# parklab/emsar

Measured on AMD Instinct MI355X. Metric: EM iterations/s, higher is better.
Workload: dtype f64

## Files before the change

### emsar_amd/csrc/emsar_hip.hip

```cpp
#include <hip/hip_runtime.h>

#include <algorithm>
#include <chrono>
#include <cmath>
#include <cstdio>
#include <cstdlib>
#include <cstring>
#include <new>
#include <numeric>
#include <string>
#include <vector>

#include "../../include/emsar_hip.h"
#include "layout.hpp"
#include "layout_tiled.hpp"
#include "sets.hpp"
#include "boot_rng.hpp"
#include "internal.hpp"
#include "devmem.hpp"
#include "fit_index.hpp"

#include "kernels_common.hpp"
#include "kernels_csr.hpp"
#include "kernels_tiled.hpp"
// ... 586 lines not shown
    return EMSAR_HIP_OK;
}

int emsar_hip_upload_euma(emsar_hip_ctx *ctx, const int32_t *euma, int32_t nfl) {
    if (!ctx || !euma || nfl <= 0) return EMSAR_HIP_ERR_ARG;
    if (!ctx->have_structure) return EMSAR_HIP_ERR_STATE;
    HIPCHK(hipSetDevice(ctx->device));
    ctx->euma = AdjEuma();
    const size_t n = (size_t)ctx->n_rows * (size_t)nfl;
    AdjEuma A;
    HIPCHK(A.d_euma_t.alloc(n));
    HIPCHK(A.d_wf.alloc((size_t)nfl));
    HIPCHK(A.d_adj.alloc((size_t)ctx->n_rows));
    if (n) {
        DevBuf<int32_t> tmp;
        HIPCHK(tmp.alloc(n));
        HIPCHK(hipMemcpyAsync(tmp, euma, n * 4, hipMemcpyHostToDevice, ctx->stream));
        dim3 grid((unsigned)((ctx->n_rows + 63) / 64), (unsigned)((nfl + 63) / 64));
        hipLaunchKernelGGL(k_transpose_i32, grid, dim3(256), 0, ctx->stream, ctx->n_rows, (int)nfl, tmp, A.d_euma_t);
        HIPCHK(hipGetLastError());
        HIPCHK(hipStreamSynchronize(ctx->stream));
    }
    A.nfl = nfl;
    ctx->euma = std::move(A);
    return EMSAR_HIP_OK;
}

int emsar_hip_adj_euma(emsar_hip_ctx *ctx, const double *wf, double *out) {
    if (!ctx || !wf || !out) return EMSAR_HIP_ERR_ARG;
    if (!ctx->have_structure || ctx->euma.nfl <= 0) return EMSAR_HIP_ERR_STATE;
    HIPCHK(hipSetDevice(ctx->device));
    if (ctx->n_rows == 0) return EMSAR_HIP_OK;
    HIPCHK(hipMemcpyAsync(ctx->euma.d_wf, wf, (size_t)ctx->euma.nfl * 8, hipMemcpyHostToDevice, ctx->stream));
    hipLaunchKernelGGL(k_adj_euma, dim3((unsigned)((ctx->n_rows + 255) / 256)), dim3(256), 0, ctx->stream, ctx->n_rows, (int)ctx->euma.nfl,
                       ctx->euma.d_euma_t, ctx->euma.d_wf, ctx->euma.d_adj);
    HIPCHK(hipGetLastError());
    HIPCHK(hipMemcpyAsync(out, ctx->euma.d_adj, (size_t)ctx->n_rows * 8, hipMemcpyDeviceToHost, ctx->stream));
    HIPCHK(hipStreamSynchronize(ctx->stream));
    return EMSAR_HIP_OK;
}

int emsar_hip_get_info(const emsar_hip_ctx *ctx, emsar_hip_info *o) {
    if (!ctx || !o) return EMSAR_HIP_ERR_ARG;
    if (!ctx->have_structure) return EMSAR_HIP_ERR_STATE;
    memset(o, 0, sizeof(*o));
    o->n_rows = ctx->n_rows; o->nnz = ctx->nnz; o->n_tx = ctx->n_tx; o->device_id = ctx->device;
    o->layout = ctx->layout | ((ctx->layout == EMSAR_LAYOUT_TILED && ctx->lay.TL.merged) ? EMSAR_LAYOUT_FLAG_MERGE_ROWS : 0);
    if (ctx->layout == EMSAR_LAYOUT_TILED) {
        o->n_chunks = ctx->lay.n_tiles; o->n_slices = ctx->tl_n_fslices; o->padded_entries = ctx->tl_fwd_slots;
        o->far_entries = ctx->lay.TL.far_entries; o->window = emsar::kTileDict;
        o->tiled_entries = ctx->lay.TL.tiled_entries; o->tiled_ids = ctx->lay.TL.tiled_ids; o->renumbered = ctx->lay.TL.renum.applied ? 1 : 0;
        o->n_units = ctx->lay.n_units;
    }
    o->bytes_per_pass = ctx->bytes_formula;
    o->stored_bytes_per_pass = stored_bytes(ctx);
    return EMSAR_HIP_OK;
}

int emsar_hip_layout_selfcheck_tiled(int64_t n_rows, int32_t n_tx, const uint64_t *row_ptr, const int32_t *col_idx,
                                     int merge_rows, emsar_hip_info *info_out) {
    try {
        if (emsar::validate_csr(n_rows, n_tx, row_ptr, col_idx) != 0) return EMSAR_HIP_ERR_ARG;
        emsar::TiledLayout L;
        if (emsar::build_tiled(n_rows, n_tx, row_ptr, col_idx, L, merge_rows != 0) != 0) return EMSAR_HIP_ERR_ARG;
        int rc = emsar::check_tiled(L, row_ptr, col_idx);
        if (rc == 0) { emsar::UnitTables U; emsar::build_unit_tables(L, U); rc = emsar::check_unit_tables(L, U); }
        if (info_out) {
            memset(info_out, 0, sizeof(*info_out));
            info_out->n_rows = n_rows; info_out->nnz = L.nnz; info_out->n_tx = n_tx;
            info_out->layout = EMSAR_LAYOUT_TILED | (L.merged ? EMSAR_LAYOUT_FLAG_MERGE_ROWS : 0);
            info_out->n_chunks = (int64_t)L.tiles.size();
            info_out->n_slices = L.n_fslices;
            info_out->padded_entries = L.padded_slots; info_out->far_entries = L.far_entries; info_out->window = emsar::kTileDict;
            info_out->stored_bytes_per_pass = (int64_t)L.fwd.size() * 4 + (int64_t)L.bwd.size() * 4 +
                                              (int64_t)L.far_tid.size() * 4 + (int64_t)L.tiles.size() * 64 + (int64_t)L.left_col.size() * 4;
            info_out->bytes_per_pass = (int64_t)L.single_row.size();
            info_out->tiled_entries = L.tiled_entries; info_out->tiled_ids = L.tiled_ids; info_out->renumbered = L.renum.applied ? 1 : 0;
            info_out->n_units = L.unit_first.empty() ? 0 : (int64_t)L.unit_first.size() - 1;
        }
        return rc == 0 ? EMSAR_HIP_OK : EMSAR_HIP_ERR_ARG - 100 + rc;
    } catch (const std::bad_alloc &) { return EMSAR_HIP_ERR_OOM; }
}

int emsar_hip_sets_selfcheck(int64_t n_rows, int32_t n_tx, const uint64_t *row_ptr, const int32_t *col_idx,
                             const int32_t *row_weight, emsar_hip_sets_info *o) {
    try {
        if (emsar::validate_csr(n_rows, n_tx, row_ptr, col_idx) != 0) return EMSAR_HIP_ERR_ARG;
        if (row_weight) for (int64_t r = 0; r < n_rows; r++) if (row_weight[r] < 0) return EMSAR_HIP_ERR_ARG;
        emsar::ResidentSets S;
        try {
            emsar::build_sets(n_rows, n_tx, row_ptr, col_idx, row_weight, S);
        } catch (const std::bad_alloc &) { return EMSAR_HIP_ERR_OOM; }
        int rc = emsar::check_sets(n_rows, n_tx, row_ptr, col_idx, row_weight, S);
        if (o) {
            memset(o, 0, sizeof(*o));
            o->n_components = S.n_components;
            for (int c = 0; c < emsar::kSetClasses; c++) { o->sets_resident[c] = (int64_t)S.desc[c].size(); o->max_lds_bytes[c] = (int64_t)S.max_lds[c]; }
            o->sets_streamed = S.n_streamed_sets;
            o->tids_closed = S.n_closed_tids; o->tids_resident = S.n_resident_tids; o->tids_streamed = S.n_streamed_tids;
            o->rows_in = S.rows_in; o->rows_stored = S.rows_stored + S.CL.rows_stored;
            o->sets_cluster = S.n_cluster_sets(); o->tids_cluster = S.CL.n_tids; o->max_lds_cluster = (int64_t)S.CL.max_lds;
        }
        return rc == 0 ? EMSAR_HIP_OK : EMSAR_HIP_ERR_ARG - 200 + rc;
    } catch (const std::bad_alloc &) { return EMSAR_HIP_ERR_OOM; }
}

}

#include "solve.hpp"
#include "resample.hpp"
#include "fit.hpp"
```

### emsar_amd/csrc/kernels_tiled.hpp

```cpp
#pragma once

namespace {

#ifndef EMSAR_UE_BATCH
#define EMSAR_UE_BATCH 6
#endif
#ifndef EMSAR_UM_BATCH
#define EMSAR_UM_BATCH 6
#endif
constexpr int kTiledThreads = 256;
constexpr int kRPL = emsar::kRowsPerLane;
constexpr int kTiledWr = emsar::kTileSliceRows + 8;
constexpr int kTiledDictPad = emsar::kDictEntries;
constexpr int kBlk = emsar::kBlk;
constexpr int kTiledLdsDoubles = 2 * kTiledDictPad + emsar::kTileSlices * kTiledWr;

__device__ __forceinline__ double lds_at(const double *base, unsigned byte_off) {
    return *reinterpret_cast<const double *>(reinterpret_cast<const char *>(base) + byte_off);
}
__device__ __forceinline__ unsigned id_off(unsigned dword, int f) { return ((dword >> (10 * f)) & 0x3FFu) << 3; }

typedef int v4i_t __attribute__((ext_vector_type(4)));
__device__ __forceinline__ void load8_clamped(int4 (&q)[8], const int4 *e, int n) {
#pragma unroll
    for (int j = 0; j < 8; j++) {
        const v4i_t t = __builtin_nontemporal_load(reinterpret_cast<const v4i_t *>(e + (size_t)(j < n ? j : n - 1) * 64));
        q[j] = make_int4(t.x, t.y, t.z, t.w);
    }
}

template <int LO>
__device__ __forceinline__ void load4_clamped(int4 (&q)[8], const int4 *e, int n) {
#pragma unroll
    for (int j = LO; j < LO + 4; j++) {
        const v4i_t t = __builtin_nontemporal_load(reinterpret_cast<const v4i_t *>(e + (size_t)(j < n ? j : n - 1) * 64));
        q[j] = make_int4(t.x, t.y, t.z, t.w);
    }
}

typedef __attribute__((address_space(3))) const double lds_cdouble;
__device__ __forceinline__ unsigned lds_byte_addr(const void *p) { return (unsigned)(uintptr_t)p; }
template <int F>
__device__ __forceinline__ unsigned lds_id_addr(unsigned dword, unsigned base ) {
    unsigned a;
    asm("v_bfe_u32 %0, %1, %2, 10\n\tv_lshl_add_u32 %0, %0, 3, %3" : "=v"(a) : "v"(dword), "i"(10 * F), "s"(base));
    return a;
}
__device__ __forceinline__ double lds_ld(unsigned a) { return *reinterpret_cast<lds_cdouble *>(a); }
template <int H>
__device__ __forceinline__ void lds_addr6(const int4 t, unsigned base, unsigned (&a)[6]) {
    const unsigned d0 = (unsigned)(H ? t.z : t.x), d1 = (unsigned)(H ? t.w : t.y);
    a[0] = lds_id_addr<0>(d0, base); a[1] = lds_id_addr<1>(d0, base); a[2] = lds_id_addr<2>(d0, base);
    a[3] = lds_id_addr<0>(d1, base); a[4] = lds_id_addr<1>(d1, base); a[5] = lds_id_addr<2>(d1, base);
}

template <int BATCH = 12, int LO = 0, int HI = 8>
__device__ __forceinline__ void fwd_sum_regs(const int4 (&q)[8], int n, unsigned th_base, double (&S)[kRPL]) {
#pragma unroll
    for (int j = LO; j < HI; j++) {
        if (j < n) {
            if (BATCH == 12) {
                unsigned a0[6], a1[6];
                double v[12];
                lds_addr6<0>(q[j], th_base, a0); lds_addr6<1>(q[j], th_base, a1);
#pragma unroll
                for (int i = 0; i < 6; i++) { v[i] = lds_ld(a0[i]); }
#pragma unroll
                for (int i = 0; i < 6; i++) { v[6 + i] = lds_ld(a1[i]); }
#pragma unroll
                for (int i = 0; i < 12; i++) S[i] += v[i];
            } else {
                unsigned a[6];
                double v[6];
                lds_addr6<0>(q[j], th_base, a);
#pragma unroll
                for (int i = 0; i < 6; i++) v[i] = lds_ld(a[i]);
#pragma unroll
                for (int i = 0; i < 6; i++) S[i] += v[i];
                lds_addr6<1>(q[j], th_base, a);
#pragma unroll
                for (int i = 0; i < 6; i++) v[i] = lds_ld(a[i]);
#pragma unroll
                for (int i = 0; i < 6; i++) S[6 + i] += v[i];
            }
        }
    }
}

__device__ __forceinline__ void tile_acc_add(double *acc_w, unsigned off, double part, double fx) {
    double *p = reinterpret_cast<double *>(reinterpret_cast<char *>(acc_w) + off);
    if (fx != 0.0) lds_add_i64(p, __double2ll_rn(part * *(p - kTiledDictPad) * fx));
    else lds_add_f64(p, part);
}
__device__ __forceinline__ void vm_loads_landed() { __builtin_amdgcn_s_waitcnt(0x0F70); }

struct DTile {
    uint64_t fwd_off, bwd_off;
    uint32_t row_base, far_off;
    int32_t lo;
    uint32_t near_n, far_n, n_slices, follows, wave_of;
    uint32_t k[4], m[4];
};
struct TileWords { uint32_t w[16]; };
static_assert(sizeof(TileWords) == sizeof(Tile), "tile_load reads a Tile as 16 dwords");
static_assert(offsetof(Tile, fwd_off) == 0 && offsetof(Tile, bwd_off) == 8 && offsetof(Tile, row_base) == 16 && offsetof(Tile, far_off) == 20 &&
              offsetof(Tile, coo_off) == 24 && offsetof(Tile, lo) == 28 && offsetof(Tile, near_n) == 32 && offsetof(Tile, far_n) == 34 &&
              offsetof(Tile, n_slices) == 36 && offsetof(Tile, follows) == 38 &&
              offsetof(Tile, wave_of) == 39 && offsetof(Tile, k) == 40 && offsetof(Tile, m) == 48 && offsetof(Tile, coo_n) == 56, "tile_load's field positions");
__device__ __forceinline__ DTile tile_load(const Tile *p ) {
    const TileWords r = *reinterpret_cast<const TileWords *>(p);
    DTile T;
    T.fwd_off = (uint64_t)r.w[0] | (uint64_t)r.w[1] << 32;
    T.bwd_off = (uint64_t)r.w[2] | (uint64_t)r.w[3] << 32;
    T.row_base = r.w[4]; T.far_off = r.w[5]; T.lo = (int32_t)r.w[7];
    T.near_n = r.w[8] & 0xFFFFu; T.far_n = r.w[8] >> 16;
    T.n_slices = r.w[9] & 0xFFFFu; T.follows = (r.w[9] >> 16) & 0xFFu; T.wave_of = r.w[9] >> 24;
#pragma unroll
    for (int s = 0; s < 4; s++) {
        T.k[s] = (r.w[10 + s / 2] >> (16 * (s & 1))) & 0xFFFFu;
        T.m[s] = (r.w[12 + s / 2] >> (16 * (s & 1))) & 0xFFFFu;
    }
    return T;
}

struct BlockDict { double th[kBlk]; int tid[kBlk]; int stid[2]; };
constexpr int kSlotsPerThread = (emsar::kTileDict + kTiledThreads - 1) / kTiledThreads;
static_assert(kSlotsPerThread <= 2, "BlockDict::stid");
static_assert(emsar::kFarMax <= kBlk * (kTiledThreads - emsar::kDictBlocks), "kBlk far entries per thread that owns no near block");
__device__ __forceinline__ void block_dict_far_issue(const int32_t *far, int n, BlockDict &D) {
#pragma unroll
    for (int i = 0; i < kBlk; i++) {
        D.tid[i] = -1;
        const int f = ((int)threadIdx.x - emsar::kDictBlocks) + i * (kTiledThreads - emsar::kDictBlocks);
        if ((int)threadIdx.x >= emsar::kDictBlocks && f < n) D.tid[i] = __builtin_nontemporal_load(&far[f]);
    }
}
template <int MODE>
__device__ __forceinline__ void block_dict_issue(const DTile &T, const double *theta, BlockDict &D) {
    const int near_n = (int)T.near_n, nb = (near_n + kBlk - 1) / kBlk;
    const bool near_thread = (int)threadIdx.x < emsar::kDictBlocks;
#pragma unroll
    for (int i = 0; i < kBlk; i++) {
        D.th[i] = 0.0;
        if (near_thread) {
            D.tid[i] = -1;
            const int d = (int)threadIdx.x * kBlk + i;
            if ((int)threadIdx.x < nb && d < near_n) D.tid[i] = T.lo + d;
        }
        if (MODE != MODE_SCATTER && D.tid[i] >= 0) D.th[i] = theta[D.tid[i]];
    }
#pragma unroll
    for (int j = 0; j < 2; j++) {
        const int sl = (int)threadIdx.x + j * kTiledThreads;
        D.stid[j] = sl < near_n ? T.lo + sl : -1;
    }
}
__device__ __forceinline__ void block_dict_store(const DTile &T, const BlockDict &D, double *th_w, double *acc_w) {
    constexpr int NE = emsar::kBlkEntries;
    const int nb = ((int)T.near_n + kBlk - 1) / kBlk;
    if ((int)threadIdx.x < emsar::kDictBlocks) {
        if ((int)threadIdx.x < nb) {
            double *t = th_w + threadIdx.x * NE, *a = acc_w + threadIdx.x * NE;
            double v[NE];
            v[0] = 0.0;
#pragma unroll
            for (int m = 1; m < NE; m++) {
                const int hi = 31 - __builtin_clz((unsigned)m);
                v[m] = v[m & ~(1 << hi)] + D.th[hi];
            }
            const int sw = EMSAR_SWZ ? (int)(threadIdx.x & (NE - 1)) : 0;
#pragma unroll
            for (int m = 0; m < NE; m++) { t[m ^ sw] = v[m]; a[m] = 0.0; }
        }
    } else {
#pragma unroll
        for (int i = 0; i < kBlk; i++) {
            if (D.tid[i] < 0) continue;
            const int e = NE * nb + ((int)threadIdx.x - emsar::kDictBlocks) + i * (kTiledThreads - emsar::kDictBlocks);
            th_w[e] = D.th[i]; acc_w[e] = 0.0;
        }
    }
}
__device__ __forceinline__ void block_dict_flush(const DTile &T, const BlockDict &D, const double *th_w, const double *acc_w, double *acc, double fx) {
    constexpr int NE = emsar::kBlkEntries;
#pragma unroll
    for (int j = 0; j < 2; j++) {
        const int tid = D.stid[j];
        if (tid < 0) continue;
        const int sl = (int)threadIdx.x + j * kTiledThreads, b = sl / kBlk, i = sl - b * kBlk;
        const double *a = acc_w + b * NE;
        const int sw = EMSAR_SWZ ? (b & (NE - 1)) : 0;
        if (fx != 0.0) {
            const double *t = th_w + b * NE;
            double si = 0.0;
#pragma unroll
            for (int m = 1; m < NE; m++) {
                const double tm = t[m ^ sw];
                if ((m >> i & 1) && tm > 0.0) si += (double)__double_as_longlong(a[m ^ sw]) / tm;
            }
            const long long iv = __double2ll_rn(t[(1 << i) ^ sw] * si);
            if (iv != 0) atomic_add_i64(&acc[tid], iv);
        } else {
            double si = 0.0;
#pragma unroll
            for (int m = 1; m < NE; m++) if (m >> i & 1) si += a[m ^ sw];
            if (si != 0.0) atomic_add_f64(&acc[tid], si);
        }
    }
#ifndef EMSAR_EXP_NO_FAR_FLUSH
    if ((int)threadIdx.x >= emsar::kDictBlocks) {
        const int nb = ((int)T.near_n + kBlk - 1) / kBlk;
#pragma unroll
        for (int i = 0; i < kBlk; i++) {
            if (D.tid[i] < 0) continue;
            const int f = ((int)threadIdx.x - emsar::kDictBlocks) + i * (kTiledThreads - emsar::kDictBlocks), e = NE * nb + f;
            const double v = acc_w[e];
            if (fx != 0.0) { const long long iv = __double_as_longlong(v); if (iv != 0) atomic_add_i64(&acc[D.tid[i]], iv); }
            else if (v != 0.0) atomic_add_f64(&acc[D.tid[i]], v);
        }
    }
#endif
}

template <int BATCH = 12, int LO = 0, int HI = 8>
__device__ __forceinline__ void bwd_sum_regs(const int4 (&q)[8], int n, unsigned ws_base, double *acc_w, unsigned &cur, double &part, double fx) {
#pragma unroll
    for (int j = LO; j < HI; j++) {
        if (j < n) {
            const unsigned col = id_off((unsigned)q[j].x, 0);
            double sum;
            if (BATCH == 12) {
                unsigned a0[6], a1[6];
                double v[12];
                lds_addr6<0>(q[j], ws_base, a0); lds_addr6<1>(q[j], ws_base, a1);
#pragma unroll
                for (int i = 1; i < 6; i++) v[i] = lds_ld(a0[i]);
#pragma unroll
                for (int i = 0; i < 6; i++) v[6 + i] = lds_ld(a1[i]);
                double s0 = v[1] + v[2], s1 = v[3] + v[4], s2 = v[5] + v[6], s3 = v[7] + v[8];
                s0 += v[9]; s1 += v[10]; s2 += v[11];
                sum = (s0 + s1) + (s2 + s3);
            } else {
                unsigned a[6];
                double v[6];
                lds_addr6<0>(q[j], ws_base, a);
#pragma unroll
                for (int i = 1; i < 6; i++) v[i] = lds_ld(a[i]);
                double s0 = v[1] + v[2], s1 = v[3] + v[4];
                s0 += v[5];
                lds_addr6<1>(q[j], ws_base, a);
#pragma unroll
                for (int i = 0; i < 6; i++) v[i] = lds_ld(a[i]);
                s0 += v[0]; s1 += v[1];
                double s2 = v[2] + v[3], s3 = v[4] + v[5];
                sum = (s0 + s1) + (s2 + s3);
            }
            if (col != cur) {
                if (part != 0.0) tile_acc_add(acc_w, cur, part, fx);
                cur = col; part = 0.0;
            }
            part += sum;
        }
    }
}

__device__ __forceinline__ unsigned long long stamp_now() {
    unsigned long long t;
    asm volatile("s_memtime %0\n\ts_waitcnt lgkmcnt(0)" : "=s"(t)::"memory");
    return t;
}

__device__ __forceinline__ unsigned long long stamp_real() {
    unsigned long long t;
    asm volatile("s_memrealtime %0\n\ts_waitcnt lgkmcnt(0)" : "=s"(t)::"memory");
    return t;
}
__device__ __forceinline__ unsigned stamp_place() {
    unsigned hw, xcc;
    asm volatile("s_getreg_b32 %0, hwreg(HW_REG_HW_ID)\n\ts_getreg_b32 %1, hwreg(HW_REG_XCC_ID)" : "=s"(hw), "=s"(xcc));
    return (xcc & 0xFu) << 16 | (hw & 0xFFFFu);
}

struct LlAcc { double v = 0.0, p = 1.0; int e = 0; };
__device__ __forceinline__ double ll_value(const LlAcc &a) { return a.v + (log(a.p) + (double)a.e * 0.6931471805599453094); }
template <int N>
__device__ __forceinline__ double sum_log_rows(const double (&S)[N], double *w_s, int lane) {
    static_assert(N == 12, "rows per lane");
    double h[2];
#pragma unroll
    for (int g = 0; g < 2; g++) {
        double p = 1.0;
#pragma unroll
        for (int i = 6 * g; i < 6 * g + 6; i++) p *= S[i] > 0.0 ? S[i] : 1.0;
        h[g] = p;
    }
    if (h[0] > 1e-140 && h[0] < 1e140 && h[1] > 1e-140 && h[1] < 1e140) return log(h[0] * h[1]);
#pragma unroll
    for (int i = 0; i < N; i++) w_s[64 * i + lane] = S[i];
    double ll = 0.0;
#pragma unroll 1
    for (int i = 0; i < N; i++) { const double v = w_s[64 * i + lane]; if (v > 0.0) ll += log(v); }
    return ll;
// ... 153 lines not shown
        const int n0 = W.k - j0 < 8 ? W.k - j0 : 8;
        if (j0) load8_clamped(A, W.e + (size_t)j0 * 64, n0);
        fwd_sum_regs<EMSAR_UE_BATCH>(A, n0, th_base, S);
    }
    if (WEIGHTED && MODE == MODE_EM_LL) {
#pragma unroll
        for (int i = 0; i < kRPL; i++) w_s[64 * i + lane] = S[i];
        __builtin_amdgcn_fence(__ATOMIC_RELEASE, "wavefront");
        double acc = 0.0;
#pragma unroll 1
        for (int i = 0; i < kRPL; i++) {
            const double s = w_s[64 * i + lane];
            const int ri = __builtin_nontemporal_load(&wgt[slot0 + 64 * i]);
            const bool live = s > 0.0 && ri > 0;
            const double rd = (double)ri;
            w_s[64 * i + lane] = live ? rd / s : 0.0;
            if (live) acc += rd * log(s);
        }
        ll.v += acc;
        __builtin_amdgcn_fence(__ATOMIC_RELEASE, "wavefront");
        __builtin_amdgcn_wave_barrier();
        __builtin_amdgcn_fence(__ATOMIC_ACQUIRE, "wavefront");
        return;
    }
    if (WEIGHTED) {
#pragma unroll
        for (int i = 0; i < kRPL; i++) r[i] = __builtin_nontemporal_load(&wgt[slot0 + 64 * i]);
    }
    if (MODE == MODE_EM_LL && !WEIGHTED) {
#pragma unroll
        for (int i = 0; i < kRPL; i++) {
            const bool pos = S[i] > 0.0;
            ll.p *= pos ? __builtin_amdgcn_frexp_mant(S[i]) : 1.0;
            ll.e += pos ? __builtin_amdgcn_frexp_exp(S[i]) : 0;
        }
        ll.e += __builtin_amdgcn_frexp_exp(ll.p);
        ll.p = __builtin_amdgcn_frexp_mant(ll.p);
    }
#pragma unroll
    for (int i = 0; i < kRPL; i++) {
        const bool live = (S[i] > 0.0) && (r[i] > 0);
        const double ri = WEIGHTED ? (double)r[i] : 1.0;
        w_s[64 * i + lane] = live ? ri / S[i] : 0.0;
        if (MODE == MODE_EM_LL && WEIGHTED && live) ll.v += ri * log(S[i]);
    }
    __builtin_amdgcn_fence(__ATOMIC_RELEASE, "wavefront");
    __builtin_amdgcn_wave_barrier();
    __builtin_amdgcn_fence(__ATOMIC_ACQUIRE, "wavefront");
}
__device__ __forceinline__ void tile_m_step(const TileWave &W, int4 (&B)[8], const double *w_s, double *acc_w, double fx) {
    const unsigned ws_base = __builtin_amdgcn_readfirstlane(lds_byte_addr(w_s));
    unsigned cur = 0xFFFFFFFFu;
    double part = 0.0;
    bwd_sum_regs<EMSAR_UM_BATCH, 0, 4>(B, W.m, ws_base, acc_w, cur, part, fx);
    if (W.m > 8) {
        const int n1 = W.m - 8 < 8 ? W.m - 8 : 8;
        const int4 *b1 = W.b + (size_t)8 * 64;
        __builtin_amdgcn_sched_barrier(0);
        load4_clamped<0>(B, b1, n1);
        __builtin_amdgcn_sched_barrier(0);
        bwd_sum_regs<EMSAR_UM_BATCH, 4, 8>(B, 8, ws_base, acc_w, cur, part, fx);
        __builtin_amdgcn_sched_barrier(0);
        load4_clamped<4>(B, b1, n1);
        __builtin_amdgcn_sched_barrier(0);
        bwd_sum_regs<EMSAR_UM_BATCH, 0, 4>(B, n1, ws_base, acc_w, cur, part, fx);
        bwd_sum_regs<EMSAR_UM_BATCH, 4, 8>(B, n1, ws_base, acc_w, cur, part, fx);
        for (int j0 = 16; j0 < W.m; j0 += 8) {
            const int n0 = W.m - j0 < 8 ? W.m - j0 : 8;
            load8_clamped(B, W.b + (size_t)j0 * 64, n0);
            bwd_sum_regs<EMSAR_UM_BATCH>(B, n0, ws_base, acc_w, cur, part, fx);
        }
    } else bwd_sum_regs<EMSAR_UM_BATCH, 4, 8>(B, W.m, ws_base, acc_w, cur, part, fx);
    if (part != 0.0) tile_acc_add(acc_w, cur, part, fx);
}
struct TileEnv {
    const Tile *tiles; int n_tiles, stride;
    const uint32_t *fwd, *bwd; const int32_t *far_tid, *wgt; const double *theta; double *acc;
    double *th_w, *acc_w, *w_s; int lane, wave; double fx;
};
template <bool WEIGHTED, int MODE, int I, int N>
__device__ __forceinline__ void tiled_stage(const TileEnv &V, int it, const DTile &T, const TileWave &W, int4 (&A)[8], int4 (&B)[8],
                                            BlockDict &D, LlAcc &ll) {
    block_dict_store(T, D, V.th_w, V.acc_w);
    const BlockDict Dcur = D;
    const int in = it + V.stride;
    const bool has_next = (I + 1 < N) && in < V.n_tiles;
    const DTile Tn = tile_load(V.tiles + (has_next ? in : it));
    __syncthreads();
    if (W.has_slice)
        tile_e_step<WEIGHTED, MODE>(W, A, (size_t)T.row_base + (size_t)V.wave * emsar::kTileSliceRows + V.lane, V.wgt, V.th_w, V.w_s, V.lane, ll);
    const TileWave Wn = tile_wave(Tn, V.wave, V.lane, V.fwd, V.bwd);
    if (has_next) {
        if (Wn.has_slice) load8_clamped(A, Wn.e, Wn.k < 8 ? Wn.k : 8);
        block_dict_far_issue(V.far_tid + Tn.far_off, (int)Tn.far_n, D);
        block_dict_issue<MODE>(Tn, V.theta, D);
    }
    if (W.has_slice) tile_m_step(W, B, V.w_s, V.acc_w, V.fx);
    if (has_next && Wn.has_slice && Wn.m > 0) load8_clamped(B, Wn.b, Wn.m < 8 ? Wn.m : 8);
    __syncthreads();
    block_dict_flush(T, Dcur, V.th_w, V.acc_w, V.acc, V.fx);
    if constexpr (I + 1 < N) {
        if (has_next) __syncthreads();
        if (has_next) tiled_stage<WEIGHTED, MODE, I + 1, N>(V, in, Tn, Wn, A, B, D, ll);
    }
}

template <bool WEIGHTED, int MODE, int N>
__global__ __launch_bounds__(kTiledThreads, 4) void k_pass_tiled_multi(const Tile *__restrict__ tiles, int n_tiles, const uint32_t *__restrict__ fwd,
                                                                    const uint32_t *__restrict__ bwd,
                                                                    const int32_t *__restrict__ far_tid, const int32_t *__restrict__ wgt,
                                                                    const double *__restrict__ theta, double *__restrict__ acc,
                                                                    double *__restrict__ ll_out, Fx fx) {
    extern __shared__ __attribute__((aligned(16))) double lds[];
    __shared__ double red[kTiledThreads / 64];
    TileEnv V;
    V.tiles = tiles; V.n_tiles = n_tiles; V.stride = (int)gridDim.x; V.fwd = fwd; V.bwd = bwd; V.far_tid = far_tid; V.wgt = wgt;
    V.theta = theta; V.acc = acc; V.fx = fx.mass;
    V.lane = threadIdx.x & 63;
    V.wave = __builtin_amdgcn_readfirstlane(threadIdx.x >> 6);
    V.th_w = lds; V.acc_w = lds + kTiledDictPad; V.w_s = lds + 2 * kTiledDictPad + V.wave * kTiledWr;
    const DTile T = tile_load(tiles + blockIdx.x);
    const TileWave W = tile_wave(T, V.wave, V.lane, fwd, bwd);
    BlockDict D;
    int4 A[8], B[8];
    block_dict_far_issue(far_tid + T.far_off, (int)T.far_n, D);
    block_dict_issue<MODE>(T, theta, D);
    if (W.has_slice) {
        load8_clamped(A, W.e, W.k < 8 ? W.k : 8);
        if (W.m > 0) load8_clamped(B, W.b, W.m < 8 ? W.m : 8);
    }
    if (V.lane < 8) V.w_s[emsar::kTileSliceRows + V.lane] = 0.0;
    LlAcc ll;
    tiled_stage<WEIGHTED, MODE, 0, N>(V, (int)blockIdx.x, T, W, A, B, D, ll);
    if (MODE == MODE_EM_LL) {
        double t = block_sum<kTiledThreads>(ll_value(ll), red);
        if (threadIdx.x == 0 && t != 0.0) ll_add(ll_out, t, fx.ll);
    }
}

template <bool WEIGHTED, int MODE, bool STAMP = false>
__global__ __launch_bounds__(kTiledThreads, 4) void k_pass_tiled_unit(const Tile *__restrict__ utiles, int stride, const int32_t *__restrict__ far_tid,
                                                                   const uint32_t *__restrict__ fwd, const uint32_t *__restrict__ bwd,
                                                                   
                                                                   const int32_t *__restrict__ wgt, const double *__restrict__ theta,
                                                                   double *__restrict__ acc, double *__restrict__ ll_out, Fx fx,
                                                                   unsigned long long *stamps = nullptr) {
    extern __shared__ __attribute__((aligned(16))) double lds[];
    __shared__ double red[kTiledThreads / 64];
    const int lane = threadIdx.x & 63;
    const int wave = __builtin_amdgcn_readfirstlane(threadIdx.x >> 6);
    double *th_w = lds, *acc_w = lds + kTiledDictPad, *w_s = lds + 2 * kTiledDictPad + wave * kTiledWr;
    unsigned long long ts0 = 0, ts1 = 0, ts2 = 0, te = 0, tm = 0, tr0 = 0;
    if (STAMP) { ts0 = stamp_now(); tr0 = stamp_real(); }
    const Tile *tiles = utiles + (size_t)blockIdx.x * (size_t)stride;
    BlockDict D;
    DTile T = tile_load(tiles);
    block_dict_far_issue(far_tid + T.far_off, (int)T.far_n, D);
    const int dict_near_n = (int)T.near_n, dict_lo = T.lo, dict_far_n = (int)T.far_n;
    const uint32_t dict_far_off = T.far_off;
    TileWave W = tile_wave(T, unit_slice(T, wave), lane, fwd, bwd);
    int4 A[8], B[8];
    load8_clamped(A, W.has_slice ? W.e : reinterpret_cast<const int4 *>(fwd), W.has_slice ? (W.k < 8 ? W.k : 8) : 1);
    block_dict_issue<MODE>(T, theta, D);
    if (lane < 8) w_s[emsar::kTileSliceRows + lane] = 0.0;
    block_dict_store(T, D, th_w, acc_w);
    vm_loads_landed();
    if (STAMP) ts1 = stamp_now();
    __syncthreads();
    if (STAMP) ts2 = stamp_now();
    LlAcc ll;
    int n_done = 0;
    for (int t = 0;; t++) {
        unsigned long long ta = 0, tb = 0;
        if (STAMP) ta = stamp_now();
        if (W.has_slice) {
            load8_clamped(B, W.b, W.m < 8 ? W.m : 8);
            tile_e_step<WEIGHTED, MODE>(W, A, (size_t)T.row_base + (size_t)W.slice * emsar::kTileSliceRows + lane, wgt, th_w, w_s, lane, ll);
        }
        const DTile Tn = tile_load(tiles + (t + 1 < stride ? t + 1 : t));
        const bool more = t + 1 < stride && Tn.n_slices > 0;
        TileWave Wn = tile_wave(Tn, unit_slice(Tn, wave), lane, fwd, bwd);
        if (!more) Wn.has_slice = false;
        if (STAMP) tb = stamp_now();
        if (W.has_slice) {
            load8_clamped(A, Wn.has_slice ? Wn.e : reinterpret_cast<const int4 *>(fwd), Wn.has_slice ? (Wn.k < 8 ? Wn.k : 8) : 1);
            tile_m_step(W, B, w_s, acc_w, fx.mass);
        } else if (Wn.has_slice) load8_clamped(A, Wn.e, Wn.k < 8 ? Wn.k : 8);
        if (STAMP) { const unsigned long long tc = stamp_now(); te += tb - ta; tm += tc - tb; }
        T = Tn; W = Wn;
        n_done = t + 1;
        if (!more) break;
    }
    unsigned long long ts3 = 0, ts4 = 0;
    if (STAMP) ts3 = stamp_now();
    block_dict_far_issue(far_tid + dict_far_off, dict_far_n, D);
    __syncthreads();
    if (STAMP) ts4 = stamp_now();
#pragma unroll
    for (int j = 0; j < 2; j++) {
        const int sl = (int)threadIdx.x + j * kTiledThreads;
        D.stid[j] = sl < dict_near_n ? dict_lo + sl : -1;
    }
    T.near_n = (uint32_t)dict_near_n;
    block_dict_flush(T, D, th_w, acc_w, acc, fx.mass);
    if (STAMP && lane == 0) {
        unsigned long long *o = stamps + ((size_t)blockIdx.x * (kTiledThreads / 64) + wave) * 8;
        o[0] = ts1 - ts0; o[1] = ts2 - ts1; o[2] = te; o[3] = tm; o[4] = ts4 - ts3; o[5] = stamp_now() - ts4; o[6] = n_done; o[7] = ts3 - ts2 - te - tm;
        if (wave == 0) {
            unsigned long long *g = stamps + (size_t)gridDim.x * (kTiledThreads / 64) * 8 + (size_t)blockIdx.x * 4;
            g[0] = tr0; g[1] = stamp_real(); g[2] = stamp_place(); g[3] = (unsigned long long)n_done;
        }
    }
    if (MODE == MODE_EM_LL) {
        double t = block_sum<kTiledThreads>(ll_value(ll), red);
        if (threadIdx.x == 0 && t != 0.0) ll_add(ll_out, t, fx.ll);
    }
}

__global__ __launch_bounds__(256) void k_single_ll(int n, const double *__restrict__ u, const double *__restrict__ theta, double *ll_out, double fx_ll) {
    __shared__ double red[4];
    double s = 0.0;
    for (int t = blockIdx.x * 256 + threadIdx.x; t < n; t += gridDim.x * 256) {
        double x = theta[t], c = u[t];
        if (c > 0.0 && x > 0.0) s += c * log(x);
    }
    double tot = block_sum<256>(s, red);
    if (threadIdx.x == 0 && tot != 0.0) ll_add(ll_out, tot, fx_ll);
}

}
```

### emsar_amd/hip.py

```python
import ctypes as C
import os

import numpy as np

_PKG = os.path.dirname(os.path.abspath(__file__))
_LIB_PATH = os.environ.get("EMSAR_HIP_LIB") or os.path.join(_PKG, "libemsar_hip.so")
_lib = None

LAYOUT_AUTO, LAYOUT_CSR, LAYOUT_TILED = 0, 1, 3
FLAG_MERGE_ROWS = 0x100

SYMBOLS = [
    "emsar_hip_create", "emsar_hip_destroy", "emsar_hip_strerror", "emsar_hip_last_error",
    "emsar_hip_upload_structure", "emsar_hip_upload_sample", "emsar_hip_solve",
    "emsar_hip_reset_theta", "emsar_hip_set_theta", "emsar_hip_get_theta", "emsar_hip_run_passes",
    "emsar_hip_ieuma", "emsar_hip_normalise", "emsar_hip_get_info",
    "emsar_hip_layout_selfcheck_tiled", "emsar_hip_sets_selfcheck", "emsar_hip_upload_euma", "emsar_hip_adj_euma", "emsar_hip_collapse_rows",
    "emsar_hip_set_deterministic", "emsar_hip_bootstrap", "emsar_hip_bootstrap_weights", "emsar_hip_bootstrap_draw_host",
    "emsar_hip_set_gene_map", "emsar_hip_gene_sums", "emsar_hip_bootstrap_genes",
    "emsar_hip_subsample", "emsar_hip_subsample_weights", "emsar_hip_subsample_draw_host",
    "emsar_hip_bootstrap_quantiles", "emsar_hip_quantiles_host",
    "emsar_hip_isoform_usage", "emsar_hip_isoform_usage_host", "emsar_hip_bootstrap_isoforms",
    "emsar_hip_model_fit", "emsar_hip_model_fit_host",
]
# ... 209 lines not shown
    return out[:, 0] if one else out


def isoform_usage_host(gene_of_tx, n_genes, cols, want_dominant=False):
    L = load_library()
    g = _arr(gene_of_tx, np.int32)
    x = _arr(cols, np.float64)
    one = x.ndim == 1
    x = np.ascontiguousarray(np.atleast_2d(x))
    if x.shape[1] != len(g):
        raise ValueError("columns of n_tx values expected")
    usage = np.zeros(x.shape)
    dom = np.zeros((x.shape[0], max(int(n_genes), 1)), dtype=np.int32) if want_dominant else None
    rc = L.emsar_hip_isoform_usage_host(len(g), int(n_genes), _p(g, C.c_int32), x.shape[0], _p(x, C.c_double), _p(usage, C.c_double),
                                        _p(dom, C.c_int32))
    if rc != 0:
        raise EmsarHipError(rc, "isoform_usage_host")
    if not want_dominant:
        return usage[0] if one else usage
    dom = dom[:, :max(int(n_genes), 0)]
    return (usage[0], dom[0]) if one else (usage, dom)


def _fit_buffers(n_rows, n_tx, n_genes, rows, genes):
    res = {k: np.zeros(max(n_tx, 1)) for k in ("tx_chi2", "tx_dev", "tx_miss", "tx_df")}
    res["tx_worst_row"] = np.zeros(max(n_tx, 1), dtype=np.int32)
    if rows:
        res.update({k: np.zeros(max(n_rows, 1)) for k in ("row_mu", "row_chi2", "row_dev")})
    if genes:
        res.update({k: np.zeros(max(n_genes, 1)) for k in ("gene_chi2", "gene_dev", "gene_miss", "gene_df")})
    o = FitOutputs()
    for k, a in res.items():
        setattr(o, k, _p(a, C.c_int32 if k == "tx_worst_row" else C.c_double))
    return res, o


def _fit_result(res, n_rows, n_tx, n_genes, st):
    out = {k: v[:(n_rows if k.startswith("row_") else n_genes if k.startswith("gene_") else n_tx)] for k, v in res.items()}
    out["stats"] = st
    return out


def model_fit_host(n_tx, row_ptr, col_idx, theta, row_weight=None, E=None, rows=False, gene_of_tx=None, n_genes=0, genes=None):
    L = load_library()
    row_ptr, col_idx, th = _arr(row_ptr, np.uint64), _arr(col_idx, np.int32), _arr(theta, np.float64)
    w, e, g = _arr(row_weight, np.int32), _arr(E, np.float64), _arr(gene_of_tx, np.int32)
    n_rows = len(row_ptr) - 1
    for a, n in ((th, n_tx), (w, n_rows), (e, n_rows), (g, n_tx)):
        if a is not None and a.shape != (n,):
            raise ValueError("array of length %d expected" % n)
    want_genes = (g is not None) if genes is None else bool(genes)
    res, o = _fit_buffers(n_rows, n_tx, int(n_genes), rows, want_genes)
    st = FitStats()
    rc = L.emsar_hip_model_fit_host(n_rows, int(n_tx), _p(row_ptr, C.c_uint64), _p(col_idx, C.c_int32), _p(w, C.c_int32), _p(e, C.c_double),
                                    _p(th, C.c_double), int(n_genes), _p(g, C.c_int32), C.byref(o), C.byref(st))
    if rc != 0:
        raise EmsarHipError(rc, "model_fit_host")
    return _fit_result(res, n_rows, int(n_tx), int(n_genes), st)


def layout_selfcheck_tiled(n_tx, row_ptr, col_idx, merge_rows=False):
    L = load_library()
    row_ptr, col_idx = _arr(row_ptr, np.uint64), _arr(col_idx, np.int32)
    info = Info()
    rc = L.emsar_hip_layout_selfcheck_tiled(len(row_ptr) - 1, n_tx, _p(row_ptr, C.c_uint64), _p(col_idx, C.c_int32),
                                            int(merge_rows), C.byref(info))
    if rc != 0:
        raise EmsarHipError(rc, "layout_selfcheck_tiled")
    d = info.as_dict()
    d["folded_single_rows"] = d.pop("bytes_per_pass")
    return d


def debug_pass_kernel(weighted, mode, n_tiles, tiled_multi=1, weighted_unit=1):
    f = load_library().emsar_hip_debug_pass_kernel
    f.argtypes = [C.c_int, C.c_int, C.c_int64, C.c_int, C.c_int, C.c_char_p, C.c_size_t]
    buf = C.create_string_buffer(64)
    rc = f(int(bool(weighted)), int(mode), int(n_tiles), int(tiled_multi), int(weighted_unit), buf, len(buf))
    if rc != 0:
        raise EmsarHipError(rc, "debug_pass_kernel")
    return buf.value.decode()


class EmsarHip:

    def __init__(self, device_id=0):
        self._L = load_library()
        h = C.c_void_p()
        rc = self._L.emsar_hip_create(C.byref(h), device_id)
        if rc != 0:
            raise EmsarHipError(rc, "emsar_hip_create")
        self._h = h
        self.n_tx = 0
        self.n_rows = 0
        self.n_genes = 0

    def close(self):
        if getattr(self, "_h", None):
            self._L.emsar_hip_destroy(self._h)
            self._h = None

    __del__ = close

    def __enter__(self):
        return self

    def __exit__(self, *a):
        self.close()

    def _chk(self, rc, what):
        if rc != 0:
            raise EmsarHipError(rc, what, self._L.emsar_hip_last_error(self._h).decode())

    def upload_structure(self, n_tx, row_ptr, col_idx, layout=LAYOUT_AUTO, merge_rows=False):
        row_ptr, col_idx = _arr(row_ptr, np.uint64), _arr(col_idx, np.int32)
        if merge_rows:
            layout |= FLAG_MERGE_ROWS
        self._chk(self._L.emsar_hip_upload_structure(self._h, len(row_ptr) - 1, n_tx, _p(row_ptr, C.c_uint64),
                                                     _p(col_idx, C.c_int32), layout), "upload_structure")
        self.n_tx = int(n_tx)
        self.n_rows = len(row_ptr) - 1
        self.n_genes = 0

    def upload_sample(self, row_weight=None, row_E=None, den=None):
        w, e, d = _arr(row_weight, np.int32), _arr(row_E, np.float64), _arr(den, np.float64)
        for a, n in ((w, self.n_rows), (e, self.n_rows), (d, self.n_tx)):
            if a is not None and a.shape != (n,):
                raise ValueError("array of length %d expected" % n)
        self._chk(self._L.emsar_hip_upload_sample(self._h, _p(w, C.c_int32), _p(e, C.c_double), _p(d, C.c_double)),
                  "upload_sample")

    def solve(self, max_iter=100000, accel=1, tol=1e-10, abs_floor=1e-6, check_every=8, count_floor=0.0, set_mode=0, zero_cut=0.0, abs_step=0.0,
              newton_after=0):
        p = EmParams(max_iter, accel, tol, abs_floor, check_every, set_mode, count_floor, zero_cut, abs_step, newton_after, 0)
        st = EmStats()
        out = np.zeros(self.n_tx)
        self._chk(self._L.emsar_hip_solve(self._h, C.byref(p), _p(out, C.c_double), C.byref(st)), "solve")
        return out, st

    def bootstrap(self, n, seed, first=0, want_replicates=False, max_iter=100000, accel=1, tol=1e-10, abs_floor=1e-6, check_every=8,
                  count_floor=0.0, set_mode=0, zero_cut=0.0, abs_step=0.0, newton_after=0):
        p = EmParams(max_iter, accel, tol, abs_floor, check_every, set_mode, count_floor, zero_cut, abs_step, newton_after, 0)
        mean, sd, tsd = np.zeros(self.n_tx), np.zeros(self.n_tx), np.zeros(self.n_tx)
        reps = np.zeros((n, self.n_tx)) if (want_replicates and n > 0) else None
        st = BootStats()
        self._chk(self._L.emsar_hip_bootstrap(self._h, C.byref(p), int(seed) & 0xFFFFFFFFFFFFFFFF, int(first), int(n), _p(mean, C.c_double),
                                              _p(sd, C.c_double), _p(tsd, C.c_double), _p(reps, C.c_double), C.byref(st)), "bootstrap")
        return mean, sd, tsd, reps, st

    def set_gene_map(self, gene_of_tx, n_genes):
        g = _arr(gene_of_tx, np.int32)
        if self.n_tx and g.shape != (self.n_tx,):
            raise ValueError("gene_of_tx must have n_tx entries")
        self._chk(self._L.emsar_hip_set_gene_map(self._h, int(n_genes), _p(g, C.c_int32)), "set_gene_map")
        self.n_genes = int(n_genes)

    def gene_sums(self, cols):
        x = _arr(cols, np.float64)
        one = x.ndim == 1
        x = np.ascontiguousarray(np.atleast_2d(x))
        if x.shape[1] != self.n_tx:
            raise ValueError("columns of n_tx values expected")
        out = np.zeros((x.shape[0], max(self.n_genes, 1)))
        self._chk(self._L.emsar_hip_gene_sums(self._h, x.shape[0], _p(x, C.c_double), _p(out, C.c_double)), "gene_sums")
        out = out[:, :self.n_genes]
        return out[0] if one else out
# ... 202 lines not shown
```

Baseline: 9695.

## Spread dictionary build across all threads with quad DPP broadcast and fold masks

Reworks the per-tile LDS dictionary build so every thread loads one near theta and up to three far entries, rather than dedicating a few threads to near blocks and the rest to far entries. Each quad of lanes shares its four thetas through DPP broadcasts and each lane writes four of the sixteen subset sums. The flush reads only the eight subset entries that contain a bit. Far tids are reloaded before the flush instead of being kept in registers across the stage. The aim is to cut the serial subset-sum work and register pressure in the build, in exchange for extra global reloads of far ids and cross-lane DPP traffic.

Measured after the change: 9806 (median of 6 runs). No clear change (+1.1%).

```diff
diff --git a/emsar_amd/csrc/dict_map.hpp b/emsar_amd/csrc/dict_map.hpp
--- /dev/null
+++ b/emsar_amd/csrc/dict_map.hpp
@@ -0,0 +1,37 @@
+#pragma once
+
+namespace emsar {
+namespace dictmap {
+
+constexpr int kThreads = 256;
+constexpr int kSlots = 4;
+constexpr int kEntries = 1 << kSlots;
+constexpr int kLaneEntries = kEntries / kSlots;
+constexpr int kFarPerThread = 3;
+constexpr int kFoldTerms = kEntries / 2;
+
+constexpr int near_blocks(int near_n) { return (near_n + kSlots - 1) / kSlots; }
+constexpr bool builds_near(int x, int nb) { return x < kSlots * nb; }
+constexpr int near_block(int x) { return x / kSlots; }
+constexpr int near_quad(int x) { return x % kSlots; }
+constexpr int built_mask(int q, int l) { return kLaneEntries * q + l; }
+constexpr int table_entry(int b, int m, int sw) { return kEntries * b + (m ^ sw); }
+
+constexpr int far_index(int x, int i) { return x + kThreads * i; }
+constexpr int far_entry(int nb, int f) { return kEntries * nb + f; }
+
+constexpr int fold_mask(int i, int c) { return ((c >> i) << (i + 1)) | (1 << i) | (c & ((1 << i) - 1)); }
+
+constexpr void quad_sums(const double (&th)[kSlots], int q, double (&v)[kLaneEntries]) {
+    const double z = 0.0, s0 = z + th[0], s1 = z + th[1], s01 = s0 + th[1];
+    v[0] = z; v[1] = s0; v[2] = s1; v[3] = s01;
+    for (int l = 0; l < kLaneEntries; l++) {
+        const double with2 = v[l] + th[2];
+        v[l] = (q & 1) ? with2 : v[l];
+        const double with3 = v[l] + th[3];
+        v[l] = (q & 2) ? with3 : v[l];
+    }
+}
+
+}
+}
diff --git a/emsar_amd/csrc/emsar_hip.hip b/emsar_amd/csrc/emsar_hip.hip
--- a/emsar_amd/csrc/emsar_hip.hip
+++ b/emsar_amd/csrc/emsar_hip.hip
@@ -692,6 +692,22 @@
     } catch (const std::bad_alloc &) { return EMSAR_HIP_ERR_OOM; }
 }
 
+int emsar_hip_debug_unit_dicts(int64_t n_rows, int32_t n_tx, const uint64_t *row_ptr, const int32_t *col_idx, int merge_rows,
+                               int32_t *out, int64_t cap, int64_t *n_units) {
+    try {
+        if (!n_units || (cap > 0 && !out) || emsar::validate_csr(n_rows, n_tx, row_ptr, col_idx) != 0) return EMSAR_HIP_ERR_ARG;
+        emsar::TiledLayout L;
+        if (emsar::build_tiled(n_rows, n_tx, row_ptr, col_idx, L, merge_rows != 0) != 0) return EMSAR_HIP_ERR_ARG;
+        const int64_t nu = L.unit_first.empty() ? 0 : (int64_t)L.unit_first.size() - 1;
+        *n_units = nu;
+        for (int64_t u = 0; u < nu && u < cap; u++) {
+            const emsar::Tile &T = L.tiles[L.unit_first[(size_t)u]];
+            out[3 * u] = T.lo; out[3 * u + 1] = (int32_t)T.near_n; out[3 * u + 2] = (int32_t)T.far_n;
+        }
+        return EMSAR_HIP_OK;
+    } catch (const std::bad_alloc &) { return EMSAR_HIP_ERR_OOM; }
+}
+
 int emsar_hip_sets_selfcheck(int64_t n_rows, int32_t n_tx, const uint64_t *row_ptr, const int32_t *col_idx,
                              const int32_t *row_weight, emsar_hip_sets_info *o) {
     try {
diff --git a/emsar_amd/csrc/kernels_tiled.hpp b/emsar_amd/csrc/kernels_tiled.hpp
--- a/emsar_amd/csrc/kernels_tiled.hpp
+++ b/emsar_amd/csrc/kernels_tiled.hpp
@@ -1,4 +1,5 @@
 #pragma once
+#include "dict_map.hpp"
 
 namespace {
 
@@ -123,101 +124,109 @@
     return T;
 }
 
-struct BlockDict { double th[kBlk]; int tid[kBlk]; int stid[2]; };
+namespace dm = emsar::dictmap;
+struct BlockDict { double th; double fth[dm::kFarPerThread]; int ftid[dm::kFarPerThread]; };
 constexpr int kSlotsPerThread = (emsar::kTileDict + kTiledThreads - 1) / kTiledThreads;
-static_assert(kSlotsPerThread <= 2, "BlockDict::stid");
-static_assert(emsar::kFarMax <= kBlk * (kTiledThreads - emsar::kDictBlocks), "kBlk far entries per thread that owns no near block");
+static_assert(kBlk == dm::kSlots && emsar::kBlkEntries == dm::kEntries && kTiledThreads == dm::kThreads, "dict_map.hpp: a block is a quad of lanes");
+static_assert(emsar::kTileDict <= kTiledThreads, "one near slot per thread in the build");
+static_assert(emsar::kFarMax <= dm::kFarPerThread * kTiledThreads, "kFarPerThread far entries per thread");
+#ifndef EMSAR_FAR_NT
+#define EMSAR_FAR_NT 3
+#endif
+template <bool NT = true>
 __device__ __forceinline__ void block_dict_far_issue(const int32_t *far, int n, BlockDict &D) {
 #pragma unroll
-    for (int i = 0; i < kBlk; i++) {
-        D.tid[i] = -1;
-        const int f = ((int)threadIdx.x - emsar::kDictBlocks) + i * (kTiledThreads - emsar::kDictBlocks);
-        if ((int)threadIdx.x >= emsar::kDictBlocks && f < n) D.tid[i] = __builtin_nontemporal_load(&far[f]);
+    for (int i = 0; i < dm::kFarPerThread; i++) {
+        D.ftid[i] = -1;
+        const int f = dm::far_index((int)threadIdx.x, i);
+        if (f < n) D.ftid[i] = NT ? __builtin_nontemporal_load(&far[f]) : far[f];
     }
 }
 template <int MODE>
 __device__ __forceinline__ void block_dict_issue(const DTile &T, const double *theta, BlockDict &D) {
-    const int near_n = (int)T.near_n, nb = (near_n + kBlk - 1) / kBlk;
-    const bool near_thread = (int)threadIdx.x < emsar::kDictBlocks;
-#pragma unroll
-    for (int i = 0; i < kBlk; i++) {
-        D.th[i] = 0.0;
-        if (near_thread) {
-            D.tid[i] = -1;
-            const int d = (int)threadIdx.x * kBlk + i;
-            if ((int)threadIdx.x < nb && d < near_n) D.tid[i] = T.lo + d;
-        }
-        if (MODE != MODE_SCATTER && D.tid[i] >= 0) D.th[i] = theta[D.tid[i]];
-    }
-#pragma unroll
-    for (int j = 0; j < 2; j++) {
+    D.th = 0.0;
+    if (MODE != MODE_SCATTER && (int)threadIdx.x < (int)T.near_n) D.th = theta[T.lo + (int)threadIdx.x];
+#pragma unroll
+    for (int i = 0; i < dm::kFarPerThread; i++) {
+        D.fth[i] = 0.0;
+        if (MODE != MODE_SCATTER && D.ftid[i] >= 0) D.fth[i] = theta[D.ftid[i]];
+    }
+}
+template <int K>
+__device__ __forceinline__ double quad_bcast(double v) {
+    constexpr int ctrl = K * 0x55;
+    const int lo = __builtin_amdgcn_update_dpp(0, __double2loint(v), ctrl, 0xF, 0xF, false);
+    const int hi = __builtin_amdgcn_update_dpp(0, __double2hiint(v), ctrl, 0xF, 0xF, false);
+    return __hiloint2double(hi, lo);
+}
+__device__ __forceinline__ void block_dict_store(const DTile &T, const BlockDict &D, double *th_w, double *acc_w) {
+    const int x = (int)threadIdx.x, nb = dm::near_blocks((int)T.near_n);
+    const double th[dm::kSlots] = {quad_bcast<0>(D.th), quad_bcast<1>(D.th), quad_bcast<2>(D.th), quad_bcast<3>(D.th)};
+    if (dm::builds_near(x, nb)) {
+        const int b = dm::near_block(x), q = dm::near_quad(x);
+        double v[dm::kLaneEntries];
+        dm::quad_sums(th, q, v);
+        const int sw = EMSAR_SWZ ? (b & (dm::kEntries - 1)) : 0;
+#pragma unroll
+        for (int l = 0; l < dm::kLaneEntries; l++) {
+            th_w[dm::table_entry(b, dm::built_mask(q, l), sw)] = v[l];
+            acc_w[dm::table_entry(b, dm::built_mask(q, l), 0)] = 0.0;
+        }
+    }
+#pragma unroll
+    for (int i = 0; i < dm::kFarPerThread; i++) {
+        if (D.ftid[i] < 0) continue;
+        const int e = dm::far_entry(nb, dm::far_index(x, i));
+        th_w[e] = D.fth[i]; acc_w[e] = 0.0;
+    }
+}
+__device__ __forceinline__ void block_dict_flush(const DTile &T, const BlockDict &D, const double *th_w, const double *acc_w, double *acc, double fx) {
+#pragma unroll
+    for (int j = 0; j < kSlotsPerThread; j++) {
         const int sl = (int)threadIdx.x + j * kTiledThreads;
-        D.stid[j] = sl < near_n ? T.lo + sl : -1;
-    }
-}
-__device__ __forceinline__ void block_dict_store(const DTile &T, const BlockDict &D, double *th_w, double *acc_w) {
-    constexpr int NE = emsar::kBlkEntries;
-    const int nb = ((int)T.near_n + kBlk - 1) / kBlk;
-    if ((int)threadIdx.x < emsar::kDictBlocks) {
-        if ((int)threadIdx.x < nb) {
-            double *t = th_w + threadIdx.x * NE, *a = acc_w + threadIdx.x * NE;
-            double v[NE];
-            v[0] = 0.0;
-#pragma unroll
-            for (int m = 1; m < NE; m++) {
-                const int hi = 31 - __builtin_clz((unsigned)m);
-                v[m] = v[m & ~(1 << hi)] + D.th[hi];
+        if (sl >= (int)T.near_n) continue;
+        const int tid = T.lo + sl, b = dm::near_block(sl), i = dm::near_quad(sl);
+        const int sw = EMSAR_SWZ ? (b & (dm::kEntries - 1)) : 0;
+        double w[dm::kFoldTerms];
+#if defined(EMSAR_EXP_FOLD_LOOP)
+        if (fx == 0.0) {
+            const double *a = acc_w + b * dm::kEntries;
+            double si = 0.0;
+#pragma unroll
+            for (int m = 1; m < dm::kEntries; m++) if (m >> i & 1) si += a[m ^ sw];
+            if (si != 0.0) atomic_add_f64(&acc[tid], si);
+            continue;
+        }
+#endif
+#pragma unroll
+        for (int c = 0; c < dm::kFoldTerms; c++) w[c] = acc_w[dm::table_entry(b, dm::fold_mask(i, c), sw)];
+        if (fx != 0.0) {
+            double t[dm::kFoldTerms];
+#pragma unroll
+            for (int c = 0; c < dm::kFoldTerms; c++) t[c] = th_w[dm::table_entry(b, dm::fold_mask(i, c), sw)];
+            double si = 0.0;
+#pragma unroll
+            for (int c = 0; c < dm::kFoldTerms; c++) {
+                const double with = si + (double)__double_as_longlong(w[c]) / t[c];
+                si = t[c] > 0.0 ? with : si;
             }
-            const int sw = EMSAR_SWZ ? (int)(threadIdx.x & (NE - 1)) : 0;
-#pragma unroll
-            for (int m = 0; m < NE; m++) { t[m ^ sw] = v[m]; a[m] = 0.0; }
-        }
-    } else {
-#pragma unroll
-        for (int i = 0; i < kBlk; i++) {
-            if (D.tid[i] < 0) continue;
-            const int e = NE * nb + ((int)threadIdx.x - emsar::kDictBlocks) + i * (kTiledThreads - emsar::kDictBlocks);
-            th_w[e] = D.th[i]; acc_w[e] = 0.0;
-        }
-    }
-}
-__device__ __forceinline__ void block_dict_flush(const DTile &T, const BlockDict &D, const double *th_w, const double *acc_w, double *acc, double fx) {
-    constexpr int NE = emsar::kBlkEntries;
-#pragma unroll
-    for (int j = 0; j < 2; j++) {
-        const int tid = D.stid[j];
-        if (tid < 0) continue;
-        const int sl = (int)threadIdx.x + j * kTiledThreads, b = sl / kBlk, i = sl - b * kBlk;
-        const double *a = acc_w + b * NE;
-        const int sw = EMSAR_SWZ ? (b & (NE - 1)) : 0;
-        if (fx != 0.0) {
-            const double *t = th_w + b * NE;
-            double si = 0.0;
-#pragma unroll
-            for (int m = 1; m < NE; m++) {
-                const double tm = t[m ^ sw];
-                if ((m >> i & 1) && tm > 0.0) si += (double)__double_as_longlong(a[m ^ sw]) / tm;
-            }
-            const long long iv = __double2ll_rn(t[(1 << i) ^ sw] * si);
+            const long long iv = __double2ll_rn(t[0] * si);
             if (iv != 0) atomic_add_i64(&acc[tid], iv);
         } else {
             double si = 0.0;
 #pragma unroll
-            for (int m = 1; m < NE; m++) if (m >> i & 1) si += a[m ^ sw];
+            for (int c = 0; c < dm::kFoldTerms; c++) si += w[c];
             if (si != 0.0) atomic_add_f64(&acc[tid], si);
         }
     }
 #ifndef EMSAR_EXP_NO_FAR_FLUSH
-    if ((int)threadIdx.x >= emsar::kDictBlocks) {
-        const int nb = ((int)T.near_n + kBlk - 1) / kBlk;
-#pragma unroll
-        for (int i = 0; i < kBlk; i++) {
-            if (D.tid[i] < 0) continue;
-            const int f = ((int)threadIdx.x - emsar::kDictBlocks) + i * (kTiledThreads - emsar::kDictBlocks), e = NE * nb + f;
-            const double v = acc_w[e];
-            if (fx != 0.0) { const long long iv = __double_as_longlong(v); if (iv != 0) atomic_add_i64(&acc[D.tid[i]], iv); }
-            else if (v != 0.0) atomic_add_f64(&acc[D.tid[i]], v);
-        }
+    const int nb = dm::near_blocks((int)T.near_n);
+#pragma unroll
+    for (int i = 0; i < dm::kFarPerThread; i++) {
+        if (D.ftid[i] < 0) continue;
+        const double v = acc_w[dm::far_entry(nb, dm::far_index((int)threadIdx.x, i))];
+        if (fx != 0.0) { const long long iv = __double_as_longlong(v); if (iv != 0) atomic_add_i64(&acc[D.ftid[i]], iv); }
+        else if (v != 0.0) atomic_add_f64(&acc[D.ftid[i]], v);
     }
 #endif
 }
@@ -537,7 +546,6 @@
 __device__ __forceinline__ void tiled_stage(const TileEnv &V, int it, const DTile &T, const TileWave &W, int4 (&A)[8], int4 (&B)[8],
                                             BlockDict &D, LlAcc &ll) {
     block_dict_store(T, D, V.th_w, V.acc_w);
-    const BlockDict Dcur = D;
     const int in = it + V.stride;
     const bool has_next = (I + 1 < N) && in < V.n_tiles;
     const DTile Tn = tile_load(V.tiles + (has_next ? in : it));
@@ -552,6 +560,8 @@
     }
     if (W.has_slice) tile_m_step(W, B, V.w_s, V.acc_w, V.fx);
     if (has_next && Wn.has_slice && Wn.m > 0) load8_clamped(B, Wn.b, Wn.m < 8 ? Wn.m : 8);
+    BlockDict Dcur;
+    block_dict_far_issue(V.far_tid + T.far_off, (int)T.far_n, Dcur);
     __syncthreads();
     block_dict_flush(T, Dcur, V.th_w, V.acc_w, V.acc, V.fx);
     if constexpr (I + 1 < N) {
@@ -610,7 +620,7 @@
     const Tile *tiles = utiles + (size_t)blockIdx.x * (size_t)stride;
     BlockDict D;
     DTile T = tile_load(tiles);
-    block_dict_far_issue(far_tid + T.far_off, (int)T.far_n, D);
+    block_dict_far_issue<(EMSAR_FAR_NT & 1) != 0>(far_tid + T.far_off, (int)T.far_n, D);
     const int dict_near_n = (int)T.near_n, dict_lo = T.lo, dict_far_n = (int)T.far_n;
     const uint32_t dict_far_off = T.far_off;
     TileWave W = tile_wave(T, unit_slice(T, wave), lane, fwd, bwd);
@@ -648,15 +658,10 @@
     }
     unsigned long long ts3 = 0, ts4 = 0;
     if (STAMP) ts3 = stamp_now();
-    block_dict_far_issue(far_tid + dict_far_off, dict_far_n, D);
+    block_dict_far_issue<(EMSAR_FAR_NT & 2) != 0>(far_tid + dict_far_off, dict_far_n, D);
     __syncthreads();
     if (STAMP) ts4 = stamp_now();
-#pragma unroll
-    for (int j = 0; j < 2; j++) {
-        const int sl = (int)threadIdx.x + j * kTiledThreads;
-        D.stid[j] = sl < dict_near_n ? dict_lo + sl : -1;
-    }
-    T.near_n = (uint32_t)dict_near_n;
+    T.near_n = (uint32_t)dict_near_n; T.lo = dict_lo;
     block_dict_flush(T, D, th_w, acc_w, acc, fx.mass);
     if (STAMP && lane == 0) {
         unsigned long long *o = stamps + ((size_t)blockIdx.x * (kTiledThreads / 64) + wave) * 8;
diff --git a/emsar_amd/hip.py b/emsar_amd/hip.py
--- a/emsar_amd/hip.py
+++ b/emsar_amd/hip.py
@@ -315,6 +315,23 @@
     return buf.value.decode()
 
 
+def debug_unit_dicts(n_tx, row_ptr, col_idx, merge_rows=False):
+    f = load_library().emsar_hip_debug_unit_dicts
+    f.argtypes = [C.c_int64, C.c_int32, C.POINTER(C.c_uint64), C.POINTER(C.c_int32), C.c_int, C.POINTER(C.c_int32), C.c_int64,
+                  C.POINTER(C.c_int64)]
+    row_ptr, col_idx = _arr(row_ptr, np.uint64), _arr(col_idx, np.int32)
+    n, out = C.c_int64(0), np.zeros((0, 3), dtype=np.int32)
+    for _ in range(2):
+        rc = f(len(row_ptr) - 1, int(n_tx), _p(row_ptr, C.c_uint64), _p(col_idx, C.c_int32), int(merge_rows), _p(out, C.c_int32),
+               len(out), C.byref(n))
+        if rc != 0:
+            raise EmsarHipError(rc, "debug_unit_dicts")
+        if len(out) == n.value:
+            break
+        out = np.zeros((n.value, 3), dtype=np.int32)
+    return out
+
+
 class EmsarHip:
 
     def __init__(self, device_id=0):
```
